# hermosayhl/CNN

Hardware: AMD Instinct MI355X
Metric: images/sec (train step, 224x224x3) (higher is better)
Workload: dtype f32; 1 GPU; reference AlexNet-style net (cpu/src/alexnet.cpp:10-33: 4x Conv3x3/s2 + ReLU, one MaxPool2x2, Linear 4608->3), full train step (fwd + softmax/CE + bwd + SGD), 224x224x3 fp32, BASELINE configs[1]; per_gpu_batch=256, global_batch=256, parallelism=dp1

## Files before the change

cnn_amd/csrc/conv_wgrad_os.hip:

```cpp
#include <cstdlib>

#include "common.h"

using namespace cnn_amd;

namespace {

typedef float f32x4 __attribute__((ext_vector_type(4)));

struct OsParams {
    const float* x;
    const float* dy;
    float* slabs;
    int B, units;
    int dbg;
};

constexpr int kCib = 16, kCob = 32;
constexpr int kWm = 3, kWn = 2, kTm = 3;
constexpr int kThreads = 64 * kWm * kWn;

template <int CI, int CO, int H, int W, int R>
struct OsGeo {
    static constexpr int Ho = (H - 3) / 2 + 1, Wo = (W - 3) / 2 + 1;
    static constexpr int XR = 2 * R + 1, XN = XR * W;
    static constexpr int PX = R * Wo, STEPS = (PX + 3) / 4;
    static constexpr int DP = ((4 * STEPS - 4 + 31) / 32) * 32 + 4;
    static constexpr int UPI = (Ho + R - 1) / R;
    static constexpr int XE = kCib * XN, DE = kCob * PX;
    static constexpr int TPX = kThreads / kCib, TPD = kThreads / kCob;
    static constexpr int NXR = (XN + TPX - 1) / TPX, NDR = (PX + TPD - 1) / TPD;
    static constexpr int PITCH = CI * 9 + 1;
    static constexpr size_t lds_bytes = (size_t)(XE + kCob * DP) * sizeof(float);
    static_assert(CI % kCib == 0 && CO % kCob == 0, "channel blocks");
    static_assert(DP >= 4 * STEPS && DP % 32 == 4, "dy pitch");
    static_assert(2 * (R - 1) + 2 < XR && 2 * (Wo - 1) + 2 < W, "window inside the staged rows");
};

template <int CI, int CO, int H, int W, int R>
__global__ __launch_bounds__(kThreads, 3) void conv_wgrad_os_kernel(const OsParams p) {
    using G = OsGeo<CI, CO, H, W, R>;
    extern __shared__ float lds[];
    float* const Xs = lds;
    float* const Ds = lds + G::XE;
    const int tid = threadIdx.x, lane = tid & 63;
    const int wave = __builtin_amdgcn_readfirstlane(tid >> 6);
    const int m = lane & 15, kq = lane >> 4;
    const int wm = wave % kWm, wn = wave / kWm;
    const int ci0 = blockIdx.y * kCib, co0 = blockIdx.z * kCob;

    for (int e = tid; e < kCob * (G::DP - G::PX); e += kThreads) {
        const int co = e / (G::DP - G::PX), off = e - co * (G::DP - G::PX);
        Ds[co * G::DP + G::PX + off] = 0.f;
    }

    int a_off[kTm];
#pragma unroll
    for (int i = 0; i < kTm; ++i) {
        const int tap = 16 * (wm * kTm + i) + m;
        a_off[i] = (tap / 9) * G::XN + ((tap % 9) / 3) * W + tap % 3;
    }
    const int b_off = (16 * wn + m) * G::DP + kq;
    int xo[G::STEPS];
#pragma unroll
    for (int j = 0; j < G::STEPS; ++j) {
        int f = 4 * j + kq;
        f = f < G::PX ? f : G::PX - 1;
        xo[j] = 2 * (f / G::Wo) * W + 2 * (f % G::Wo);
    }

    f32x4 acc[kTm];
#pragma unroll
    for (int i = 0; i < kTm; ++i) acc[i] = f32x4{0.f, 0.f, 0.f, 0.f};
    float bsum = 0.f;

    float xr[G::NXR], dr[G::NDR];
    const int sci = tid / G::TPX, sxo = tid - sci * G::TPX;
    const int sco = tid / G::TPD, sdo = tid - sco * G::TPD;
    float* const xs_w = Xs + sci * G::XN + sxo;
    float* const ds_w = Ds + sco * G::DP + sdo;
    auto fetch = [&](int u) {
        const int b = u / G::UPI, r0 = (u - b * G::UPI) * R;
        const float* xb = p.x + ((size_t)b * CI + ci0 + sci) * (H * W) + 2 * r0 * W + sxo;
        const float* db = p.dy + ((size_t)b * CO + co0 + sco) * (G::Ho * G::Wo) + r0 * G::Wo + sdo;
        const int xlim = ((H - 2 * r0) * W < G::XN ? (H - 2 * r0) * W : G::XN) - sxo;
        const int dlim = ((G::Ho - r0) * G::Wo < G::PX ? (G::Ho - r0) * G::Wo : G::PX) - sdo;
#pragma unroll
        for (int i = 0; i < G::NXR; ++i) xr[i] = i * G::TPX < xlim ? xb[i * G::TPX] : 0.f;
#pragma unroll
        for (int i = 0; i < G::NDR; ++i) dr[i] = i * G::TPD < dlim ? db[i * G::TPD] : 0.f;
    };
    auto commit = [&]() {
#pragma unroll
        for (int i = 0; i < G::NXR; ++i)
            if (sxo + i * G::TPX < G::XN) xs_w[i * G::TPX] = xr[i];
#pragma unroll
        for (int i = 0; i < G::NDR; ++i)
            if (sdo + i * G::TPD < G::PX) ds_w[i * G::TPD] = dr[i];
    };

    int u = blockIdx.x;
    if (u < p.units) fetch(u);
    for (; u < p.units; u += gridDim.x) {
        __syncthreads();
        commit();
        __syncthreads();
        const int un = u + gridDim.x;
        if (un < p.units && p.dbg != 1) fetch(un);
        if (p.dbg == 2) continue;
        const int r0 = (u % G::UPI) * R;
        const int rows = G::Ho - r0 < R ? G::Ho - r0 : R;
        const int pxv = rows * G::Wo;
#pragma unroll
        for (int j = 0; j < G::STEPS; ++j) {
            const float bv = Ds[b_off + 4 * j];
            const bool live = 4 * j + kq < pxv;
            float av[kTm];
#pragma unroll
            for (int i = 0; i < kTm; ++i) {
                const float v = Xs[a_off[i] + xo[j]];
                av[i] = live ? v : 0.f;
            }
#pragma unroll
            for (int i = 0; i < kTm; ++i) acc[i] = __builtin_amdgcn_mfma_f32_16x16x4f32(av[i], bv, acc[i], 0, 0, 0);
            bsum += bv;
        }
    }

    float* slab = p.slabs + (size_t)blockIdx.x * CO * G::PITCH;
    const int co = co0 + 16 * wn + m;
#pragma unroll
    for (int i = 0; i < kTm; ++i)
#pragma unroll
        for (int r = 0; r < 4; ++r) {
            const int tap = ci0 * 9 + 16 * (wm * kTm + i) + 4 * kq + r;
            slab[(size_t)co * G::PITCH + tap] = acc[i][r];
        }
    if (blockIdx.y == 0 && wm == 0) {
        float v = bsum;
        v += __shfl_xor(v, 16, 64);
        v += __shfl_xor(v, 32, 64);
        if (kq == 0) slab[(size_t)co * G::PITCH + CI * 9] = v;
    }
}

struct OsShape {
    int Ci, Co, H, W, slots;
};
constexpr OsShape kShapes[] = {{16, 32, 55, 55, 512}, {32, 64, 27, 27, 128}, {64, 128, 13, 13, 32}};

const OsShape* find_shape(const cnn_conv2d_desc* d) {
    const bool off = (CNN_OPT_SET("WGRAD_OS") && CNN_OPT_INT("WGRAD_OS", 0) == 0);
    if (off || d->k != 3 || d->s != 2 || d->pad != 0 || d->B < 1) return nullptr;
    const int mask = CNN_OPT_INT("WGRAD_OS_MASK", 5);
    int bit = 1;
    for (const OsShape& s : kShapes) {
        if ((mask & bit) && d->Ci == s.Ci && d->Co == s.Co && d->H == s.H && d->W == s.W) return &s;
        bit <<= 1;
    }
    return nullptr;
}

template <int CI, int CO, int H, int W, int R>
int launch_os(const cnn_conv2d_desc* d, const float* x, const float* dy, float* slabs, int slots, hipStream_t s) {
    using G = OsGeo<CI, CO, H, W, R>;
    OsParams p;
    p.x = x; p.dy = dy; p.slabs = slabs; p.B = d->B;
    p.units = d->B * G::UPI;
    p.dbg = CNN_MEASURE_INT("OS_DBG", 0);
    static DeviceOnce attr_once;
    if (attr_once.needed()) {
        CNN_HIP_CHECK(hipFuncSetAttribute((const void*)conv_wgrad_os_kernel<CI, CO, H, W, R>, hipFuncAttributeMaxDynamicSharedMemorySize,
                                          (int)G::lds_bytes));
        attr_once.mark();
    }
    const dim3 grid((unsigned)slots, CI / kCib, CO / kCob);
    char name[48];
    snprintf(name, sizeof(name), "conv_wgrad_os<%d,%d>", CI, CO);
    CNN_KLAUNCH(s, name, (conv_wgrad_os_kernel<CI, CO, H, W, R><<<grid, kThreads, G::lds_bytes, s>>>(p)),
                "B%d Ci%d %dx%d Co%d k3 s2 p0 slabs%d", d->B, CI, H, W, CO, slots);
    return CNN_AMD_OK;
}

}

namespace cnn_amd {

int os_wgrad_slots(const cnn_conv2d_desc* d) {
    const OsShape* sh = find_shape(d);
    if (!sh) return 0;
    int slots = sh->slots;
    if (const OptVal e = CNN_OPT_VAL("OS_SLABS")) {
        const int v = atoi(e);
        if (v > 0) slots = v;
    }
    const OptVal per = sh->H == 55 ? CNN_OPT_VAL("OS_SLABS2") : (sh->H == 27 ? CNN_OPT_VAL("OS_SLABS3") : CNN_OPT_VAL("OS_SLABS4"));
    if (per && atoi(per) > 0) slots = atoi(per);
    const int upi = sh->H == 55 ? 9 : (sh->H == 27 ? 2 : 1);
    const long long units = (long long)d->B * upi;
    if (units >= (1ll << 30)) return 0;
    return slots < units ? slots : (int)units;
}

int os_wgrad_launch(const cnn_conv2d_desc* d, const float* x, const float* dy, float* slabs, hipStream_t s) {
    const int slots = os_wgrad_slots(d);
    CNN_REQUIRE(slots > 0, "os_wgrad_launch: geometry not covered");
    if (d->Ci == 16) return launch_os<16, 32, 55, 55, 3>(d, x, dy, slabs, slots, s);
    if (d->Ci == 32) return launch_os<32, 64, 27, 27, 7>(d, x, dy, slabs, slots, s);
    return launch_os<64, 128, 13, 13, 6>(d, x, dy, slabs, slots, s);
}

}
```

Measured before the change: 647,400 images/sec.

## Deepen wgrad prefetch pipeline with register-depth slots and double-buffered LDS

```diff
diff --git a/cnn_amd/csrc/conv_wgrad_os.hip b/cnn_amd/csrc/conv_wgrad_os.hip
--- a/cnn_amd/csrc/conv_wgrad_os.hip
+++ b/cnn_amd/csrc/conv_wgrad_os.hip
@@ -1,4 +1,5 @@
 #include <cstdlib>
+#include <type_traits>
 
 #include "common.h"
 
@@ -28,30 +29,50 @@
     static constexpr int DP = ((4 * STEPS - 4 + 31) / 32) * 32 + 4;
     static constexpr int UPI = (Ho + R - 1) / R;
     static constexpr int XE = kCib * XN, DE = kCob * PX;
-    static constexpr int TPX = kThreads / kCib, TPD = kThreads / kCob;
-    static constexpr int NXR = (XN + TPX - 1) / TPX, NDR = (PX + TPD - 1) / TPD;
+    static constexpr int NX = (XE + kThreads - 1) / kThreads, ND = (DE + kThreads - 1) / kThreads;
     static constexpr int PITCH = CI * 9 + 1;
-    static constexpr size_t lds_bytes = (size_t)(XE + kCob * DP) * sizeof(float);
+    static constexpr int BUF = XE + kCob * DP;
+    static constexpr size_t lds_bytes = (size_t)BUF * sizeof(float);
+    static constexpr bool kTwoBuf = 2 * lds_bytes <= 32 * 1024;
+    static constexpr bool kPartial = Ho % R != 0 || (H - 2 * (UPI - 1) * R) * W < XN;
     static_assert(CI % kCib == 0 && CO % kCob == 0, "channel blocks");
     static_assert(DP >= 4 * STEPS && DP % 32 == 4, "dy pitch");
     static_assert(2 * (R - 1) + 2 < XR && 2 * (Wo - 1) + 2 < W, "window inside the staged rows");
 };
 
-template <int CI, int CO, int H, int W, int R>
+template <int N, int LIMIT>
+struct FlatDiv {
+    static constexpr unsigned kShift = 24, kMul = ((1u << kShift) + N - 1) / N;
+    static constexpr bool exact() {
+        for (unsigned e = 0; e < (unsigned)LIMIT; ++e)
+            if (((e * kMul) >> kShift) != e / N) return false;
+        return true;
+    }
+    static_assert(kMul < (1u << 24) && (unsigned long long)LIMIT * kMul < (1ull << 32) && exact(), "FlatDiv: multiplier not exact on the range");
+    __device__ static __forceinline__ unsigned div(unsigned e) { return __umul24(e, kMul) >> kShift; }
+};
+
+template <int N, int I = 0, typename F>
+__device__ __forceinline__ void for_slots(F&& f) {
+    if constexpr (I < N) {
+        f(std::integral_constant<int, I>());
+        for_slots<N, I + 1>(f);
+    }
+}
+
+template <int CI, int CO, int H, int W, int R, int D, bool TWO>
 __global__ __launch_bounds__(kThreads, 3) void conv_wgrad_os_kernel(const OsParams p) {
     using G = OsGeo<CI, CO, H, W, R>;
     extern __shared__ float lds[];
-    float* const Xs = lds;
-    float* const Ds = lds + G::XE;
     const int tid = threadIdx.x, lane = tid & 63;
     const int wave = __builtin_amdgcn_readfirstlane(tid >> 6);
     const int m = lane & 15, kq = lane >> 4;
     const int wm = wave % kWm, wn = wave / kWm;
     const int ci0 = blockIdx.y * kCib, co0 = blockIdx.z * kCob;
 
-    for (int e = tid; e < kCob * (G::DP - G::PX); e += kThreads) {
-        const int co = e / (G::DP - G::PX), off = e - co * (G::DP - G::PX);
-        Ds[co * G::DP + G::PX + off] = 0.f;
+    for (int e = tid; e < (TWO ? 2 : 1) * kCob * (G::DP - G::PX); e += kThreads) {
+        const int row = e / (G::DP - G::PX), off = e - row * (G::DP - G::PX);
+        lds[(row / kCob) * G::BUF + G::XE + (row % kCob) * G::DP + G::PX + off] = 0.f;
     }
 
     int a_off[kTm];
@@ -60,7 +81,7 @@
         const int tap = 16 * (wm * kTm + i) + m;
         a_off[i] = (tap / 9) * G::XN + ((tap % 9) / 3) * W + tap % 3;
     }
-    const int b_off = (16 * wn + m) * G::DP + kq;
+    const int b_off = G::XE + (16 * wn + m) * G::DP + kq;
     int xo[G::STEPS];
 #pragma unroll
     for (int j = 0; j < G::STEPS; ++j) {
@@ -74,56 +95,108 @@
     for (int i = 0; i < kTm; ++i) acc[i] = f32x4{0.f, 0.f, 0.f, 0.f};
     float bsum = 0.f;
 
-    float xr[G::NXR], dr[G::NDR];
-    const int sci = tid / G::TPX, sxo = tid - sci * G::TPX;
-    const int sco = tid / G::TPD, sdo = tid - sco * G::TPD;
-    float* const xs_w = Xs + sci * G::XN + sxo;
-    float* const ds_w = Ds + sco * G::DP + sdo;
-    auto fetch = [&](int u) {
+    float xr[D][G::NX], dr[D][G::ND];
+    auto fetch = [&](int u, bool live, float (&xv)[G::NX], float (&dv)[G::ND]) {
+        u = live ? u : (int)blockIdx.x;
         const int b = u / G::UPI, r0 = (u - b * G::UPI) * R;
-        const float* xb = p.x + ((size_t)b * CI + ci0 + sci) * (H * W) + 2 * r0 * W + sxo;
-        const float* db = p.dy + ((size_t)b * CO + co0 + sco) * (G::Ho * G::Wo) + r0 * G::Wo + sdo;
-        const int xlim = ((H - 2 * r0) * W < G::XN ? (H - 2 * r0) * W : G::XN) - sxo;
-        const int dlim = ((G::Ho - r0) * G::Wo < G::PX ? (G::Ho - r0) * G::Wo : G::PX) - sdo;
-#pragma unroll
-        for (int i = 0; i < G::NXR; ++i) xr[i] = i * G::TPX < xlim ? xb[i * G::TPX] : 0.f;
-#pragma unroll
-        for (int i = 0; i < G::NDR; ++i) dr[i] = i * G::TPD < dlim ? db[i * G::TPD] : 0.f;
+        const float* xb = p.x + ((size_t)b * CI + ci0) * (H * W) + 2 * r0 * W;
+        const float* db = p.dy + ((size_t)b * CO + co0) * (G::Ho * G::Wo) + r0 * G::Wo;
+        const unsigned xlim = !live ? 0 : ((H - 2 * r0) * W < G::XN ? (H - 2 * r0) * W : G::XN);
+        const unsigned dlim = !live ? 0 : ((G::Ho - r0) * G::Wo < G::PX ? (G::Ho - r0) * G::Wo : G::PX);
+        unsigned t = tid;
+        asm volatile("" : "+v"(t));
+#pragma unroll
+        for (int i = 0; i < G::NX; ++i) {
+            const unsigned e = t + i * kThreads, c = FlatDiv<G::XN, G::NX * kThreads>::div(e), off = e - c * G::XN;
+            const bool ok = e < (unsigned)G::XE && off < xlim;
+            xv[i] = xb[ok ? c * (H * W) + off : 0u];
+        }
+#pragma unroll
+        for (int i = 0; i < G::ND; ++i) {
+            const unsigned e = t + i * kThreads, c = FlatDiv<G::PX, G::ND * kThreads>::div(e), off = e - c * G::PX;
+            const bool ok = e < (unsigned)G::DE && off < dlim;
+            dv[i] = db[ok ? c * (G::Ho * G::Wo) + off : 0u];
+        }
     };
-    auto commit = [&]() {
-#pragma unroll
-        for (int i = 0; i < G::NXR; ++i)
-            if (sxo + i * G::TPX < G::XN) xs_w[i * G::TPX] = xr[i];
-#pragma unroll
-        for (int i = 0; i < G::NDR; ++i)
-            if (sdo + i * G::TPD < G::PX) ds_w[i * G::TPD] = dr[i];
+    auto commit = [&](const float (&xv)[G::NX], const float (&dv)[G::ND], float* buf, int u) {
+        unsigned xlim = G::XN, dlim = G::PX;
+        if constexpr (G::kPartial) {
+            const int r0 = (u % G::UPI) * R;
+            xlim = (H - 2 * r0) * W < G::XN ? (H - 2 * r0) * W : G::XN;
+            dlim = (G::Ho - r0) * G::Wo < G::PX ? (G::Ho - r0) * G::Wo : G::PX;
+        }
+#pragma unroll
+        for (int i = 0; i < G::NX; ++i) {
+            const unsigned e = tid + i * kThreads;
+            float v = xv[i];
+            if constexpr (G::kPartial) v = e - (e / G::XN) * G::XN < xlim ? v : 0.f;
+            if (e < (unsigned)G::XE) buf[e] = v;
+        }
+#pragma unroll
+        for (int i = 0; i < G::ND; ++i) {
+            const unsigned e = tid + i * kThreads, c = e / G::PX, off = e - c * G::PX;
+            float v = dv[i];
+            if constexpr (G::kPartial) v = off < dlim ? v : 0.f;
+            if (e < (unsigned)G::DE) buf[G::XE + c * G::DP + off] = v;
+        }
     };
-
-    int u = blockIdx.x;
-    if (u < p.units) fetch(u);
-    for (; u < p.units; u += gridDim.x) {
-        __syncthreads();
-        commit();
-        __syncthreads();
-        const int un = u + gridDim.x;
-        if (un < p.units && p.dbg != 1) fetch(un);
-        if (p.dbg == 2) continue;
+    auto mfma_unit = [&](int u, const float* buf) {
         const int r0 = (u % G::UPI) * R;
         const int rows = G::Ho - r0 < R ? G::Ho - r0 : R;
         const int pxv = rows * G::Wo;
 #pragma unroll
         for (int j = 0; j < G::STEPS; ++j) {
-            const float bv = Ds[b_off + 4 * j];
+            const float bv = buf[b_off + 4 * j];
             const bool live = 4 * j + kq < pxv;
             float av[kTm];
 #pragma unroll
             for (int i = 0; i < kTm; ++i) {
-                const float v = Xs[a_off[i] + xo[j]];
+                const float v = buf[a_off[i] + xo[j]];
                 av[i] = live ? v : 0.f;
             }
 #pragma unroll
             for (int i = 0; i < kTm; ++i) acc[i] = __builtin_amdgcn_mfma_f32_16x16x4f32(av[i], bv, acc[i], 0, 0, 0);
             bsum += bv;
+        }
+    };
+
+    const int step = gridDim.x;
+    int u = blockIdx.x;
+    auto has = [&](int un) { return un < p.units && p.dbg != 1; };
+    for_slots<D>([&](auto K) {
+        constexpr int k = decltype(K)::value;
+        const int uk = u + k * step;
+        fetch(uk, k == 0 ? uk < p.units : has(uk), xr[k], dr[k]);
+    });
+    if constexpr (!TWO) {
+        while (u < p.units) {
+            for_slots<D>([&](auto K) {
+                constexpr int k = decltype(K)::value;
+                if (u >= p.units) return;
+                __syncthreads();
+                commit(xr[k], dr[k], lds, u);
+                __syncthreads();
+                fetch(u + D * step, has(u + D * step), xr[k], dr[k]);
+                if (p.dbg != 2) mfma_unit(u, lds);
+                u += step;
+            });
+        }
+    } else {
+        int par = 0;
+        commit(xr[0], dr[0], lds, u);
+        fetch(u + D * step, has(u + D * step), xr[0], dr[0]);
+        __syncthreads();
+        while (u < p.units) {
+            for_slots<D>([&](auto K) {
+                constexpr int k = decltype(K)::value, kn = (k + 1) % D;
+                if (u >= p.units) return;
+                if (p.dbg != 2) mfma_unit(u, lds + par * G::BUF);
+                par ^= 1;
+                commit(xr[kn], dr[kn], lds + par * G::BUF, u + step);
+                fetch(u + (D + 1) * step, has(u + (D + 1) * step), xr[kn], dr[kn]);
+                __syncthreads();
+                u += step;
+            });
         }
     }
 
@@ -161,6 +234,23 @@
     return nullptr;
 }
 
+constexpr int kMaxDepth = 3, kDefaultDepth = 2;
+
+template <int CI, int CO, int H, int W, int R, int D>
+int launch_os_d(const OsParams& p, const dim3 grid, const char* name, const cnn_conv2d_desc* d, hipStream_t s) {
+    using G = OsGeo<CI, CO, H, W, R>;
+    constexpr bool TWO = D > 1 && G::kTwoBuf;
+    constexpr size_t lds = (TWO ? 2 : 1) * G::lds_bytes;
+    auto kern = conv_wgrad_os_kernel<CI, CO, H, W, R, D, TWO>;
+    static DeviceOnce attr_once;
+    if (attr_once.needed()) {
+        CNN_HIP_CHECK(hipFuncSetAttribute((const void*)kern, hipFuncAttributeMaxDynamicSharedMemorySize, (int)lds));
+        attr_once.mark();
+    }
+    CNN_KLAUNCH(s, name, (kern<<<grid, kThreads, lds, s>>>(p)), "B%d Ci%d %dx%d Co%d k3 s2 p0 slabs%d", d->B, CI, H, W, CO, (int)grid.x);
+    return CNN_AMD_OK;
+}
+
 template <int CI, int CO, int H, int W, int R>
 int launch_os(const cnn_conv2d_desc* d, const float* x, const float* dy, float* slabs, int slots, hipStream_t s) {
     using G = OsGeo<CI, CO, H, W, R>;
@@ -168,18 +258,15 @@
     p.x = x; p.dy = dy; p.slabs = slabs; p.B = d->B;
     p.units = d->B * G::UPI;
     p.dbg = CNN_MEASURE_INT("OS_DBG", 0);
-    static DeviceOnce attr_once;
-    if (attr_once.needed()) {
-        CNN_HIP_CHECK(hipFuncSetAttribute((const void*)conv_wgrad_os_kernel<CI, CO, H, W, R>, hipFuncAttributeMaxDynamicSharedMemorySize,
-                                          (int)G::lds_bytes));
-        attr_once.mark();
-    }
     const dim3 grid((unsigned)slots, CI / kCib, CO / kCob);
     char name[48];
     snprintf(name, sizeof(name), "conv_wgrad_os<%d,%d>", CI, CO);
-    CNN_KLAUNCH(s, name, (conv_wgrad_os_kernel<CI, CO, H, W, R><<<grid, kThreads, G::lds_bytes, s>>>(p)),
-                "B%d Ci%d %dx%d Co%d k3 s2 p0 slabs%d", d->B, CI, H, W, CO, slots);
-    return CNN_AMD_OK;
+    int depth = CNN_OPT_INT("OS_DEPTH", kDefaultDepth);
+    depth = depth < 1 ? 1 : (depth > kMaxDepth ? kMaxDepth : depth);
+    if (depth == 1) return launch_os_d<CI, CO, H, W, R, 1>(p, grid, name, d, s);
+    if (depth == 2) return launch_os_d<CI, CO, H, W, R, 2>(p, grid, name, d, s);
+    if constexpr (G::NX + G::ND + G::STEPS > 46) return launch_os_d<CI, CO, H, W, R, 2>(p, grid, name, d, s);
+    else return launch_os_d<CI, CO, H, W, R, 3>(p, grid, name, d, s);
 }
 
 }
```

Result: slower. 608,300 images/sec (-6.0%).
